# albertfgu/diffwave-sashimi

Hardware: AMD Instinct MI355X
Metric: audio samples/sec (generate.py-style reverse-diffusion sampling, T=200) (higher is better)
Workload: dtype f32-equivalent (3-term bf16 split, 6 products, fp32 accumulate); 1 GPU; wnet_h256_d36_T200; backbone=wavenet, batch_per_gpu=16, L=16000, T=200, parallelism=independent clips per GPU, no collective, sampler=hipGraph replay, on-device Philox noise

## Files before the change

diffwave-sashimi_amd/csrc/wavenet.h:

```cpp
#pragma once
#include "dws_common.h"

namespace dws {

constexpr int WN_LAYER_KC = 32;
constexpr int WN_BX3_KC = 16;

struct WnLayerArgs {
    const float* x_in;
    float* x_out;
    float* skip;
    const float* part_t;
    int part_t_bstride;
    const float* A1;
    const float* A2;
    const float* Abt;
    int abt_bstride;
    const int* step_idx;
    int abt_tstride, part_t_tstride;
    const float* Wd;
    const float* Wr;
    const float* Ws;
    const float* bias1;
    const float* bias2;
// ... 18 lines not shown
    float scale;
    int B, L, Cout;
    int af_scaled;
};

int launch_fold_weight_norm(const float* v, const float* g, float* out, int O, int inner, hipStream_t s);
int launch_permute_dconv(const float* w, float* out, int C, int KC, hipStream_t s);
int launch_pack_a_frag(const float* w, float* out, int M, int K, hipStream_t s);
int launch_pack_a_frag_t(const float* w, float* out, int O, int K, hipStream_t s);
int launch_step_embed(const float* steps, const float* freq, float* emb, int B, int half, hipStream_t s);
int launch_iota_f32(float* out, int n, hipStream_t s);
int launch_linear_rows(const float* in, const float* W, const float* bias, float* out, int B, int K, int O,
                       int act, hipStream_t s, float* pre_out = nullptr);
int launch_init_conv_bwd_data(const float* g, const float* y, const float* W, float* daudio, int B, int Cin, int C, int L,
                              hipStream_t s);
int launch_init_conv(const float* audio, const float* W, const float* bias, float* x, int B, int Cin, int C, int L,
                     hipStream_t s);
int launch_wn_bias_tap(const float* Wd_all, const float* part_t, float* Abt, int NL, int B, int C, hipStream_t s);
bool wn_layer_mfma_supported(int C, int S);
int launch_wn_layer_mfma(int C, int S, const WnLayerArgs& a, hipStream_t s);
int launch_wn_layer_generic(int C, int S, const WnLayerArgs& a, hipStream_t s);
bool wn_final_mfma_supported(int S);
bool wn_layer_wino_supported(int C, int S);
int launch_wino_dconv(const float* w, float* out, int C, hipStream_t s);
int launch_wn_wino_bias(const float* Wd_all, const float* part_t, float* Abt, int NL, int B, int C, hipStream_t s);
int launch_wn_layer_wino(int C, int S, const WnLayerArgs& a, hipStream_t s);
bool wn_layer_bf16x3_supported(int C, int S);
int launch_wn_layer_bf16x3(int C, int S, const WnLayerArgs& a, hipStream_t s);
int launch_pack_a_bf16x3(const float* w, void* out, int M, int K, hipStream_t s);
int launch_wn_bias_tap_bf16(const float* Wd_all, const float* part_t, const float* bias1_all, void* Abt, int NL, int B, int C,
                            hipStream_t s);
enum { WN_SPLIT_BF16X6 = 0, WN_SPLIT_F16X3 = 1 };
inline int wn_split_terms(int split) { return split == WN_SPLIT_F16X3 ? 2 : 3; }
enum { WN_BX6_MFMA_32 = 0, WN_BX6_MFMA_G2_16 = 1, WN_BX6_MFMA_16 = 2 };
constexpr int WN_BX6_MFMA_DEFAULT = WN_BX6_MFMA_16;
bool wn_layer_bx6_supported(int C, int S);
bool wn_layer_bx6_mfma16_supported(int C, int S, int split);
int launch_wn_layer_bx6(int C, int S, const WnLayerArgs& a, int split, int mfma, hipStream_t s);
int launch_weight_scale(const float* w, size_t n, const float* bias, int nb, const float* bias_b, int nb_b, float* out, hipStream_t s);
int launch_pack_a1_bx6(const float* w, void* out, int C, int split, const float* scale, hipStream_t s);
int launch_pack_a_bx6(const float* w, void* out, int M, int K, int split, const float* scale, hipStream_t s);
int launch_gemm_bx6(const float* A, const float* B, float* C, int M, int N, int K, int split, float sa, float sb, hipStream_t s);
int launch_wn_final(int S, const WnFinalArgs& a, hipStream_t s);

}
```

diffwave-sashimi_amd/csrc/wavenet_bx6.hip:

```cpp
#include <cstdlib>
#include <type_traits>

#include "bf16_split.h"
#include "wavenet.h"
#include "wn_trace.h"

namespace dws {

#ifndef BX6_PF3
#define BX6_PF3 1
#endif
#ifndef BX6_PF2
#define BX6_PF2 2
#endif
#define BX6_PF(NT) ((NT) == 2 ? BX6_PF2 : BX6_PF3)
#ifndef BX6_T_SLOTS
#define BX6_T_SLOTS 0, 2, 3, 4, 6, 7, 9
#endif

typedef float bx6_f32x4 __attribute__((ext_vector_type(4)));

#ifdef BX6_ABL_NO_NT
#define BX6_NT 0
#else
// ... 102 lines not shown
    if (split == WN_SPLIT_F16X3) {
        DWS_CHECK(scale != nullptr, DWS_ERR_INVALID, "pack_a: the fp16 split needs the matrix scale");
        hipLaunchKernelGGL(pack_a_bx6_kernel<SplitF16x2>, dim3(ceil_div(n, 256)), dim3(256), 0, s, w, (unsigned short*)out, M, K, scale);
    } else {
        hipLaunchKernelGGL(pack_a_bx6_kernel<SplitBf16x3>, dim3(ceil_div(n, 256)), dim3(256), 0, s, w, (unsigned short*)out, M, K, scale);
    }
    return DWS_OK;
}

template <int C, int S, int NT>
struct Bx6Tile {
    static constexpr int WAVES = C / 32;
    static constexpr int NTH = WAVES * 64;
    static constexpr int NP = 32;
    static constexpr int KC = (C >= 256) ? 32 : 16;
    static constexpr int NCB = C / KC;
    static constexpr int NKB = C / 16;
    static constexpr int MS = S / C;
    static constexpr int RAW_FLOATS = KC * 4 * NP;
    static constexpr int BOP_BYTES = (KC / 8) * 4 * NT * NP * 16;
    static constexpr int STAGE_FLOATS = 2 * RAW_FLOATS + 2 * BOP_BYTES / 4;
    static constexpr int GATE_BYTES = (C / 8) * NT * 64 * 16;
    static constexpr int MAIN_FLOATS = STAGE_FLOATS > GATE_BYTES / 4 ? STAGE_FLOATS : GATE_BYTES / 4;
    static constexpr int TR_FLOATS = 32 * 64;
    static constexpr int LDS_FLOATS = MAIN_FLOATS + WAVES * TR_FLOATS;
    static constexpr int TITEMS = (KC / 4) * NP * 2;
    static constexpr bool HALVES = WAVES == 8 && NT == 3;
    static constexpr int SW = HALVES ? WAVES / 2 : WAVES;
    static constexpr int NPIECE = KC / (2 * SW);
    static_assert(C % 32 == 0 && S % C == 0 && C % KC == 0 && KC % 16 == 0 && KC % (2 * SW) == 0 && (SW & (SW - 1)) == 0 &&
                  (!HALVES || NCB % 2 == 0) && (TITEMS % NTH == 0) && LDS_FLOATS * 4 <= 163840, "channel counts");
};

enum { BX6_MF_32 = 0, BX6_MF_G2_16 = 1, BX6_MF_16 = 2 };
#ifndef BX6_T16_SLOTS
#define BX6_T16_SLOTS 1, 5, 7, 9, 13, 15, 19
#endif
struct Bx6Nothing {};
template <int MS>
struct Bx6G2State {
    float bias[1 + MS][2];
    bx_f32x4 acc[1 + MS][2][2][2];
};
template <int NT>
__device__ __forceinline__ int bx6_voff_a1h(int lane) { return ((lane >> 5) * (4 * NT * 64) + ((lane >> 4) & 1) * 32 + (lane & 15)) * 16; }
template <typename V8, int NT>
__device__ __forceinline__ void bx6_load_a1h(V8 (&dst)[2][NT], __amdgpu_buffer_rsrc_t r, int voff, int soff) {
#pragma unroll
    for (int h = 0; h < 2; ++h)
#pragma unroll
        for (int t = 0; t < NT; ++t) dst[h][t] = __builtin_bit_cast(V8, __builtin_amdgcn_raw_buffer_load_b128(r, voff + h * 256, soff + t * 1024, 0));
}
template <typename V8, int NT>
struct Bx6G1State {
    float av[2][2][4], ab[2][2];
    bx_f32x4 acc[2][4][2][2];
    V8 ar[2][2][NT];
    int pc[2];
};
template <typename P, int C, int S, bool EXTRA, int MF = BX6_MF_32>
__global__ __launch_bounds__(C * 2, (C >= 128 ? 2 : 1)) void wn_layer_bx6_kernel(WnLayerArgs a, int log2d) {
    using T = Bx6Tile<C, S, P::NT>;
    static_assert(MF == BX6_MF_32 || (P::NT == 3 && !P::SCALED && C == 256 && S == 256), "the 16x16x32 shape: bf16 split, C = S = 256");
    using v8 = typename P::v8;
    using v4 = typename P::v4;
    constexpr int NT = P::NT, NPR = P::NP, NA = 2 * P::NT;
    constexpr int KC = T::KC, MS = T::MS, WAVES = T::WAVES, NCB = T::NCB, NTH = T::NTH, NKB = T::NKB;
    __shared__ __attribute__((aligned(16))) float lds[T::LDS_FLOATS];
    float* const Xraw = lds;
    char* const Bop = reinterpret_cast<char*>(lds + 2 * T::RAW_FLOATS);
    char* const gt = reinterpret_cast<char*>(lds);

    const int tid = threadIdx.x;
    const int lane = tid & 63;
    const int wave = __builtin_amdgcn_readfirstlane(tid >> 6);
    const int l31 = lane & 31, lhi = lane >> 5;
    const int L = a.L, dil = 1 << log2d;
    float* const trw = lds + T::MAIN_FLOATS + wave * T::TR_FLOATS;

    const int nblk = (L + 2 * dil - 1) >> (log2d + 1);
    const int ntl = ((nblk << log2d) + 31) >> 5;
    const int tile = xcd_remap(blockIdx.x, gridDim.x);
    const int b = __builtin_amdgcn_readfirstlane(tile / ntl);
    const int tic = tile % ntl;
#ifdef WN_TILE_ORDER_LINEAR
    const int q0 = __builtin_amdgcn_readfirstlane(tic * 32);
#else
    const int q0 = __builtin_amdgcn_readfirstlane(log2d >= 6 ? ((tic % nblk) << log2d) + (tic / nblk) * 32 : tic * 32);
#endif
    const int q = q0 + l31;
    const int p = ((q >> log2d) << (log2d + 1)) + (q & (dil - 1));

    const float* __restrict__ xb = a.x_in + (size_t)b * C * L;
    unsigned long long* __restrict__ trc = a.trace ? a.trace + ((size_t)blockIdx.x * WAVES + wave) * 32 : nullptr;
    auto stamp = [&](int i) {
        if (trc) {
            const unsigned long long t = __builtin_amdgcn_s_memtime();
            if (lane == 0) trc[i] = t;
        }
    };
// ... 132 lines not shown
#pragma unroll
                for (int e = 0; e < 2; ++e) {
                    const float da = ts.d[k][e][0], d1 = ts.d[k][e][1], d2 = ts.d[k][e][2];
                    if (w == 1) t4[2 * h + e] = (p1 ? d2 : da) - (p1 ? d1 : d2);
                    else t4[2 * h + e] = d1 + (p1 ? -da : d2);
                    if (P::SCALED) t4[2 * h + e] *= P::SX;
                }
                v4 q[NT];
                P::split4(t4, q);
#pragma unroll
                for (int t = 0; t < NT; ++t)
#pragma unroll
                    for (int e = 2 * h; e < 2 * h + 2; ++e) {
                        if (w == 1) ts.pa[k][t][e] = q[t][e];
                        else ts.pb[k][t][e] = q[t][e];
                    }
            }
        }
    };
    auto transform = [&](int c1) {
        TState ts;
#pragma unroll
        for (int u = 0; u < T_UNITS; ++u) transform_unit(c1, u, ts);
    };
    auto keep_residual = [&](int c1) {
        const int ch0 = chunk_of(c1) * KC;
        if (al16 && ch0 / 32 == wave) {
            const float* xs = Xraw + (c1 & 1) * T::RAW_FLOATS;
            const int r0 = ch0 % 32;
#pragma unroll
            for (int i = 0; i < KC / 4; ++i) {
                const int rr = (lane >> 4) + 4 * i;
                const bx6_f32x4 v = *reinterpret_cast<const bx6_f32x4*>(xs + rr * 128 + 32 + 4 * (lane & 15));
                *reinterpret_cast<bx6_f32x4*>(trw + (r0 + rr) * 64 + 4 * (lane & 15)) = v;
            }
        }
    };

    bx_f32x16 acc[2][4];
    __amdgpu_buffer_rsrc_t rA1 = __builtin_amdgcn_make_buffer_rsrc((void*)a.A1, 0, 2 * C * 4 * C * 2 * NT, 0x00020000);
    const int lane16 = lane * 16;
    auto load_a1 = [&](v8 (&dst)[2][NT], int kb, int j) {
#pragma unroll
        for (int m = 0; m < 2; ++m)
#pragma unroll
            for (int t = 0; t < NT; ++t)
#ifdef BX6_ABL_A_HOT
                dst[m][t] = __builtin_bit_cast(v8, __builtin_amdgcn_raw_buffer_load_b128(rA1, lane16, ((mt1[m] * NKB * 4) * NT + t) * 1024 + 0 * (kb + j), 0));
#else
                dst[m][t] = __builtin_bit_cast(v8, __builtin_amdgcn_raw_buffer_load_b128(rA1, lane16, (((mt1[m] * NKB + kb) * 4 + j) * NT + t) * 1024, 0));
#endif
    };

    if (stages(0)) stage_dma(0);
    if (NCB > 1 && stages(1)) stage_dma(1);
    constexpr int PF = BX6_PF(NT);
    v8 a_ring[4][2][NT];
    if constexpr (MF >= BX6_MF_16) {
        static_assert(MF < BX6_MF_16 || (PF == 1 && KC == 32), "one half-step of six fragments ahead: NAF and every vmcnt count as in the 32x32x16 form");
        bx6_load_a1h<v8, NT>(gs1.ar[0], rA1, bx6_voff_a1h<NT>(lane), ((mt1[0] * NKB + 2 * chunk_of(0)) * 4 + 0) * NT * 1024);
    } else {
#pragma unroll
    for (int s0 = 0; s0 < PF; ++s0) load_a1(a_ring[s0], chunk_of(0) * (KC / 16) + (s0 >> 2), s0 & 3);
    }
    constexpr int NAF = PF * NA;
    constexpr int P16 = NPIECE + NAF, P4 = 4 * NPIECE + NAF;
    static_assert(P4 < 64, "vmcnt is a 6-bit counter");
// ... 207 lines not shown
    }
    }
    stamp(2);
    int lane_t = lane;
    if constexpr (MF >= BX6_MF_16) asm volatile("" : "+v"(lane_t));

    [[maybe_unused]] std::conditional_t<MF >= BX6_MF_G2_16, Bx6G2State<MS>, Bx6Nothing> gs2;
    if constexpr (MF >= BX6_MF_G2_16) {
#pragma unroll
        for (int m = 0; m < 1 + MS; ++m)
#pragma unroll
            for (int h = 0; h < 2; ++h) gs2.bias[m][h] = a.bias2[mt2[m] * 32 + 16 * h + (lane_t & 15)];
    }
    const int L4 = L * 4;
    const bool first = a.first_layer, last = a.last_layer;
    __amdgpu_buffer_rsrc_t rXo = __builtin_amdgcn_make_buffer_rsrc((void*)(a.x_out + (size_t)b * C * L), 0, C * L * 4, 0x00020000);
    __amdgpu_buffer_rsrc_t rSk = __builtin_amdgcn_make_buffer_rsrc((void*)(a.skip + (size_t)b * S * L), 0, S * L * 4, 0x00020000);
    const int p0 = ((q0 >> log2d) << (log2d + 1)) + (q0 & (dil - 1));
    int voff4;
    {
        const int n4 = (lane_t & 15) >> 3;
        const int pos4 = (contig ? pbase + 32 * n4 : p0 + n4 * dil) + 4 * (lane_t & 7);
        voff4 = (pos4 < L) ? ((lane_t >> 4) * L + pos4) * 4 : 0x7ffffff0;
    }
    constexpr bool PRELOAD = MS == 1;
    const int voff4s = first ? 0x7ffffff0 : voff4;
    auto load_pre = [&](int m, bx6_f32x4 (&dst)[8]) {
#pragma unroll
        for (int i = 0; i < 8; ++i) {
            if (m == 0) dst[i] = *reinterpret_cast<const bx6_f32x4*>(trw + ((lane_t >> 4) + 4 * i) * 64 + 4 * (lane_t & 15));
            else dst[i] = bx6_load_f4(rSk, voff4s, ((wave * MS + (m - 1)) * 32 + 4 * i) * L4);
        }
    };
    bx6_f32x4 pre[PRELOAD ? 1 + MS : 1][8];
    if (PRELOAD && al16) {
#pragma unroll
        for (int m = 1; m < 1 + MS; ++m) load_pre(m, pre[PRELOAD ? m : 0]);
    }

    const float* melb = (EXTRA && a.melc) ? a.melc + (size_t)(a.mel_bstride ? b : 0) * 2 * C * L : nullptr;
    if constexpr (MF >= BX6_MF_16) {
        const int r16 = lane_t & 15, oct = lane_t >> 4;
#pragma unroll
        for (int c = 0; c < 2; ++c) {
            const int qc = q0 + 16 * c + r16;
            const int pc = ((qc >> log2d) << (log2d + 1)) + (qc & (dil - 1));
            const int gc0 = contig ? pc - pbase : 16 * c + r16, gc1 = contig ? pc - pbase + dil : 32 + 16 * c + r16;
#pragma unroll
            for (int h = 0; h < 2; ++h) {
                float ga[4], gb[4];
#pragma unroll
                for (int e = 0; e < 4; ++e) {
                    const int ch = wave * 32 + 16 * h + 4 * oct + e;
#pragma unroll
                    for (int n = 0; n < 2; ++n) {
                        const int pos = pc + n * dil;
                        float ht, hs;
                        if (n == 0) {
                            ht = (gs1.acc[0][0][h][c][e] + gs1.acc[0][1][h][c][e]) + gs1.acc[0][2][h][c][e];
                            hs = (gs1.acc[1][0][h][c][e] + gs1.acc[1][1][h][c][e]) + gs1.acc[1][2][h][c][e];
                        } else {
                            ht = (gs1.acc[0][1][h][c][e] - gs1.acc[0][2][h][c][e]) - gs1.acc[0][3][h][c][e];
                            hs = (gs1.acc[1][1][h][c][e] - gs1.acc[1][2][h][c][e]) - gs1.acc[1][3][h][c][e];
                        }
                        if (EXTRA && melb && pos < L) {
                            ht += melb[(size_t)ch * L + pos];
                            hs += melb[(size_t)(C + ch) * L + pos];
                        }
// ... 107 lines not shown
            v8 bq[2][NT];
#pragma unroll
            for (int n = 0; n < 2; ++n)
#pragma unroll
                for (int t = 0; t < NT; ++t) bq[n][t] = *reinterpret_cast<const v8*>(gk + (t * 64 + n * 32) * 16);
#pragma unroll
            for (int t = 0; t < NPR; ++t)
#pragma unroll
                for (int m = M0; m < 1 + MS; ++m)
#pragma unroll
                    for (int n = 0; n < 2; ++n)
                        acc2[m][n] = P::mfma(c_cur[m][P::ia(t)], bq[n][P::ib(t)], acc2[m][n]);
#pragma unroll
            for (int m = M0; m < 1 + MS; ++m)
#pragma unroll
                for (int t = 0; t < NT; ++t) c_cur[m][t] = c_nxt[m][t];
        }
    };
    if constexpr (MF >= BX6_MF_G2_16) {
        auto gemm2_16 = [&](auto WITH_RES) {
            const int r16 = lane_t & 15, oct = lane_t >> 4;
            auto& acc2h = gs2.acc;
            constexpr int M0 = decltype(WITH_RES)::value ? 0 : 1;
            const int voffa = (oct >> 1) * (NT * 1024) + ((oct & 1) * 32 + r16) * 16;
            auto load_a2h = [&](v8 (&dst)[1 + MS][NT], int kk, int h) {
#pragma unroll
                for (int m = M0; m < 1 + MS; ++m)
#pragma unroll
                    for (int t = 0; t < NT; ++t)
                        dst[m][t] = __builtin_bit_cast(v8, __builtin_amdgcn_raw_buffer_load_b128(rA2, voffa + h * 256, ((mt2[m] * NKB + 2 * kk) * NT + t) * 1024, 0));
            };
            auto block_of = [&](int kk) { const int k = kk + rot; return k >= NCB ? k - NCB : k; };
            static_assert(KC == 32, "GEMM2's rotation counts 32-channel blocks");
            v8 ah[2][1 + MS][NT];
            load_a2h(ah[0], block_of(0), 0);
            {
                const v8 bf = P::bvals_16(P::SG, 0.f, lane_t);
                const bx_f32x4 zero = {0.f, 0.f, 0.f, 0.f};
#pragma unroll
                for (int m = M0; m < 1 + MS; ++m)
#pragma unroll
                    for (int h = 0; h < 2; ++h) {
                        v8 af[NT];
                        P::rank2_16(gs2.bias[m][h] * ws2, 0.f, lane_t, af);
#pragma unroll
                        for (int n = 0; n < 2; ++n)
#pragma unroll
                            for (int c = 0; c < 2; ++c) {
                                acc2h[m][n][h][c] = zero;
#pragma unroll
                                for (int t = NT - 1; t >= 0; --t) acc2h[m][n][h][c] = P::mfma16(af[t], bf, acc2h[m][n][h][c]);
                            }
                    }
            }
            __syncthreads();
            stamp(4);
            const char* gb = gt + oct * (NT * 64 * 16) + r16 * 16;
#pragma unroll 1
            for (int kk = 0; kk < NCB; ++kk) {
                const char* gk = gb + block_of(kk) * (4 * NT * 64 * 16);
                v8 bq[2][2][NT];
#pragma unroll
                for (int h = 0; h < 2; ++h) {
                    if (h == 0) load_a2h(ah[1], block_of(kk), 1);
                    else load_a2h(ah[0], block_of(kk + 1 < NCB ? kk + 1 : kk), 0);
                    __builtin_amdgcn_sched_barrier(0);
                    if (h == 0) {
#pragma unroll
                        for (int n = 0; n < 2; ++n)
#pragma unroll
                            for (int c = 0; c < 2; ++c)
#pragma unroll
                                for (int t = 0; t < NT; ++t) bq[n][c][t] = *reinterpret_cast<const v8*>(gk + (t * 64 + n * 32 + c * 16) * 16);
                    }
#pragma unroll
                    for (int t = 0; t < NPR; ++t)
#pragma unroll
                        for (int m = M0; m < 1 + MS; ++m)
#pragma unroll
                            for (int n = 0; n < 2; ++n)
#pragma unroll
                                for (int c = 0; c < 2; ++c)
                                    acc2h[m][n][h][c] = P::mfma16(ah[h][m][P::ia(t)], bq[n][c][P::ib(t)], acc2h[m][n][h][c]);
                }
            }
        };
        if (last) gemm2_16(std::false_type{});
        else gemm2_16(std::true_type{});
    } else {
        if (last) gemm2(std::false_type{});
        else gemm2(std::true_type{});
    }
    stamp(5);

    const float rs = 0.70710678118654752440f;
    if (al16) {
#pragma unroll
        for (int m = 0; m < 1 + MS; ++m) {
            if (m == 0 && last) continue;
            if (!PRELOAD || m == 0) load_pre(m, pre[0]);
            asm volatile("s_waitcnt lgkmcnt(0)" ::: "memory");
            if constexpr (MF >= BX6_MF_G2_16) {
                const int r16 = lane_t & 15, oct = lane_t >> 4;
                auto& acc2h = gs2.acc;
#pragma unroll
                for (int n = 0; n < 2; ++n)
#pragma unroll
                    for (int h = 0; h < 2; ++h)
#pragma unroll
                        for (int c = 0; c < 2; ++c)
#pragma unroll
                            for (int r = 0; r < 4; ++r) trw[(16 * h + 4 * oct + r) * 64 + ((n * 32 + 16 * c + r16) ^ (oct << 4))] = acc2h[m][n][h][c][r];
            } else {
#pragma unroll
            for (int n = 0; n < 2; ++n)
#pragma unroll
                for (int r = 0; r < 16; ++r) trw[((r & 3) + 8 * (r >> 2) + 4 * lhi) * 64 + n * 32 + l31] = P::SCALED ? acc2[m][n][r] * inv2 : acc2[m][n][r];
            }
            asm volatile("s_waitcnt lgkmcnt(0)" ::: "memory");
            const int row0 = (m == 0) ? wave * 32 : (wave * MS + (m - 1)) * 32;
#pragma unroll
            for (int i = 0; i < 8; ++i) {
                const bx6_f32x4 v = *reinterpret_cast<const bx6_f32x4*>(trw + ((lane_t >> 4) + 4 * i) * 64 +
                                                                        (MF >= BX6_MF_G2_16 ? (4 * (lane_t & 15)) ^ ((i & 3) << 4) : 4 * (lane_t & 15)));
                bx6_f32x4 o = pre[PRELOAD ? m : 0][i] + v;
                if (m == 0) o = o * rs;
                bx6_store_f4(o, m == 0 ? rXo : rSk, voff4, (row0 + 4 * i) * L4);
                asm volatile("s_nop 1" ::: "memory");
            }
// ... 91 lines not shown
    else hipLaunchKernelGGL((wn_layer_bx6_kernel<P, C, S, false, MF>), dim3(ntiles), dim3(T::NTH), 0, s, a, log2d);
    return DWS_OK;
}

bool wn_layer_bx6_mfma16_supported(int C, int S, int split) { return split == WN_SPLIT_BF16X6 && C == 256 && S == 256; }

bool wn_layer_bx6_supported(int C, int S) {
    return (C == 64 && S == 64) || (C == 128 && S == 128) || (C == 128 && S == 256) || (C == 256 && S == 256);
}

template <typename P>
static int launch_bx6_p(int C, int S, const WnLayerArgs& a, int log2d, hipStream_t s) {
    if (C == 64 && S == 64) return launch_bx6_t<P, 64, 64>(a, log2d, s);
    if (C == 128 && S == 128) return launch_bx6_t<P, 128, 128>(a, log2d, s);
    if (C == 128 && S == 256) return launch_bx6_t<P, 128, 256>(a, log2d, s);
    if (C == 256 && S == 256) return launch_bx6_t<P, 256, 256>(a, log2d, s);
    return set_error(DWS_ERR_UNSUPPORTED, "wn_layer_bx6: (C=%d,S=%d) not instantiated", C, S);
}

int launch_wn_layer_bx6(int C, int S, const WnLayerArgs& a, int split, int mfma, hipStream_t s) {
    int log2d = 0;
    while ((1 << log2d) < a.dilation) ++log2d;
    DWS_CHECK((1 << log2d) == a.dilation, DWS_ERR_UNSUPPORTED, "wn_layer_bx6: dilation %d is not a power of two", a.dilation);
    DWS_CHECK((int64_t)a.L + 4 * (int64_t)a.dilation < ((int64_t)1 << 28), DWS_ERR_UNSUPPORTED, "wn_layer_bx6: L too large");
    DWS_CHECK((int64_t)(C > S ? C : S) * a.L * 4 < ((int64_t)1 << 31), DWS_ERR_UNSUPPORTED,
              "wn_layer_bx6: %d channels x L=%d exceed a 2 GiB tensor per clip", C > S ? C : S, a.L);
    if (split == WN_SPLIT_F16X3) {
        DWS_CHECK(a.hsave == nullptr, DWS_ERR_UNSUPPORTED, "wn_layer_f16x3: the training forward runs with precision=f32 or bf16x6");
        DWS_CHECK(a.wscale != nullptr, DWS_ERR_INVALID, "wn_layer_f16x3: no weight scales");
        return launch_bx6_p<SplitF16x2>(C, S, a, log2d, s);
    }
    if (mfma == WN_BX6_MFMA_G2_16 && wn_layer_bx6_mfma16_supported(C, S, split)) return launch_bx6_t<SplitBf16x3, 256, 256, BX6_MF_G2_16>(a, log2d, s);
    if (mfma == WN_BX6_MFMA_16 && wn_layer_bx6_mfma16_supported(C, S, split)) return launch_bx6_t<SplitBf16x3, 256, 256, BX6_MF_16>(a, log2d, s);
    DWS_CHECK(mfma == WN_BX6_MFMA_32 || mfma == WN_BX6_MFMA_G2_16 || mfma == WN_BX6_MFMA_16, DWS_ERR_INVALID, "wn_layer_bx6: unknown MFMA shape %d", mfma);
    return launch_bx6_p<SplitBf16x3>(C, S, a, log2d, s);
}

template <typename P>
__global__ __launch_bounds__(64) void gemm_bx6_kernel(const float* __restrict__ A, const float* __restrict__ B, float* __restrict__ Cm,
                                                      int M, int N, int K, float sa, float sb) {
    using v8 = typename P::v8;
    const int lane = threadIdx.x, l31 = lane & 31, lhi = lane >> 5;
    const int mt = blockIdx.y, nt = blockIdx.x;
    bx_f32x16 acc;
#pragma unroll
    for (int r = 0; r < 16; ++r) acc[r] = 0.f;
    for (int kb = 0; kb < K / 16; ++kb) {
        v8 af[P::NT], bf[P::NT];
#pragma unroll
        for (int e = 0; e < 8; ++e) {
            const int k = kb * 16 + 8 * lhi + e;
            P::split1(A[(size_t)(mt * 32 + l31) * K + k] * sa, af, e);
            P::split1(B[(size_t)k * N + nt * 32 + l31] * sb, bf, e);
        }
#pragma unroll
        for (int t = 0; t < P::NP; ++t) acc = P::mfma(af[P::ia(t)], bf[P::ib(t)], acc);
    }
    const float inv = 1.f / (sa * sb);
#pragma unroll
    for (int r = 0; r < 16; ++r)
        Cm[(size_t)(mt * 32 + (r & 3) + 8 * (r >> 2) + 4 * lhi) * N + nt * 32 + l31] = acc[r] * inv;
}

int launch_gemm_bx6(const float* A, const float* B, float* Cm, int M, int N, int K, int split, float sa, float sb, hipStream_t s) {
    DWS_CHECK(M > 0 && N > 0 && K > 0 && M % 32 == 0 && N % 32 == 0 && K % 16 == 0, DWS_ERR_UNSUPPORTED,
              "gemm_bf16x6 / gemm_f16x3: M=%d N=%d must be multiples of 32, K=%d of 16", M, N, K);
    if (split == WN_SPLIT_F16X3) {
// ... 25 lines not shown
```

diffwave-sashimi_amd/csrc/wavenet_kernels.hip:

```cpp
#include "dws_common.h"
#include "model.h"
#include "wavenet.h"

namespace dws {

typedef float f32x16 __attribute__((ext_vector_type(16)));


__device__ __forceinline__ void fold_weight_norm_row(const float* __restrict__ v, const float* __restrict__ g,
                                                     float* __restrict__ out, int inner, int o, float* red) {
    const float* vr = v + (size_t)o * inner;
    float s = 0.f;
    for (int i = threadIdx.x; i < inner; i += 256) s += vr[i] * vr[i];
    red[threadIdx.x] = s;
    __syncthreads();
    for (int st = 128; st > 0; st >>= 1) {
        if (threadIdx.x < st) red[threadIdx.x] += red[threadIdx.x + st];
        __syncthreads();
    }
    const float scale = g[o] / sqrtf(red[0]);
    for (int i = threadIdx.x; i < inner; i += 256) out[(size_t)o * inner + i] = vr[i] * scale;
}

__global__ __launch_bounds__(256) void fold_weight_norm_kernel(const float* __restrict__ v, const float* __restrict__ g,
// ... 185 lines not shown
#pragma unroll
        for (int off = 32; off > 0; off >>= 1) acc += __shfl_xor(acc, off);
        if (lane == 0) {
            float y = acc + bo;
            if (pre_out) pre_out[(size_t)b * O + o] = y;
            if (ACT == 1) y = y / (1.f + expf(-y));
            out[(size_t)b * O + o] = y;
        }
    }
}

int launch_linear_rows(const float* in, const float* W, const float* bias, float* out, int B, int K, int O,
                       int act, hipStream_t s, float* pre_out) {
    DWS_CHECK(K <= 1024, DWS_ERR_UNSUPPORTED, "linear_rows: K=%d > 1024 not supported", K);
    dim3 grid(ceil_div(O, 4)), block(256);
    if (act == 1)
        hipLaunchKernelGGL(linear_rows_kernel<1>, grid, block, 0, s, in, W, bias, out, B, K, O, pre_out);
    else
        hipLaunchKernelGGL(linear_rows_kernel<0>, grid, block, 0, s, in, W, bias, out, B, K, O, pre_out);
    return DWS_OK;
}

__global__ void init_conv_kernel(const float* __restrict__ audio, const float* __restrict__ W,
                                 const float* __restrict__ bias, float* __restrict__ x, int Cin, int C, int L) {
    const int b = blockIdx.z, c = blockIdx.y;
    const float bc = bias[c];
    for (int l = blockIdx.x * blockDim.x + threadIdx.x; l < L; l += gridDim.x * blockDim.x) {
        float acc = bc;
        for (int ci = 0; ci < Cin; ++ci) acc = fmaf(W[c * Cin + ci], audio[((size_t)b * Cin + ci) * L + l], acc);
        x[((size_t)b * C + c) * L + l] = dws_relu(acc);
    }
}

int launch_init_conv(const float* audio, const float* W, const float* bias, float* x, int B, int Cin, int C, int L,
                     hipStream_t s) {
    ProfileScope ps("init_conv", s);
    dim3 grid(min(ceil_div(L, 256), 64), C, B);
    hipLaunchKernelGGL(init_conv_kernel, grid, dim3(256), 0, s, audio, W, bias, x, Cin, C, L);
    return DWS_OK;
}

__global__ __launch_bounds__(64) void wn_mask_tail_kernel(float* __restrict__ x, const int32_t* __restrict__ lengths,
                                                          const float* __restrict__ pt, int pt_bstride,
                                                          const int* __restrict__ step_idx, int pt_tstride, int C, int L,
                                                          int reach, size_t row_stride, int div) {
    const int b = blockIdx.y, c = blockIdx.x, lane = threadIdx.x;
    const int len = min(max(lengths[b] / div, 0), L);
    const int end = reach < 0 ? L : (int)min((int64_t)L, (int64_t)len + reach);
    if (len >= end) return;
    const float v = pt ? -pt[(size_t)b * pt_bstride + c + step_row_off(step_idx, pt_tstride)] : 0.f;
    float* row = x + ((size_t)b * C + c) * row_stride;
    const int head = (int)((4 - (((uintptr_t)(row + len) >> 2) & 3)) & 3);
    const int a0 = min(len + head, end);
    const int nvec = (end - a0) >> 2;
    for (int i = len + lane; i < a0; i += 64) row[i] = v;
    float4* q = reinterpret_cast<float4*>(row + a0);
    const float4 v4 = make_float4(v, v, v, v);
    for (int k = lane; k < nvec; k += 64) q[k] = v4;
    for (int i = a0 + 4 * nvec + lane; i < end; i += 64) row[i] = v;
}

int launch_wn_mask_tail(float* x, const int32_t* lengths, int B, int C, int L, int reach, const float* pt, int pt_bstride,
                        const int* step_idx, int pt_tstride, hipStream_t s) {
    ProfileScope ps("wn_mask_tail", s);
    DWS_CHECK(B >= 1 && B <= 65535, DWS_ERR_UNSUPPORTED, "per-clip lengths: B = %d (the grid has one row per clip: 1 .. 65535)", B);
    hipLaunchKernelGGL(wn_mask_tail_kernel, dim3(C, B), dim3(64), 0, s, x, lengths, pt, pt_bstride, step_idx, pt_tstride, C, L, reach,
                       (size_t)L, 1);
    return DWS_OK;
}
// ... 607 lines not shown
```

diffwave-sashimi_amd/csrc/wavenet_model.hip:

```cpp
#include <cmath>

#include "conditioner.h"
#include "model.h"
#include "wavenet.h"
#include "wavenet_backward.h"

namespace dws {

struct WaveNetModel : dws_model {
    int Cin, Cout, C, S, NL, cycle, Ein, Emid, Eout, MB;
    bool cond, mfma_layer, mfma_final;
    bool bf16x3 = false;
    bool bf16x6 = false;
    bool f16x3 = false;
    DevBuf wscale;
    bool wino_opt = true;
    int bx6_mfma = WN_BX6_MFMA_DEFAULT;
    bool bx6_mfma_env_bad = false;
    static bool parse_bx6_mfma(const std::string& v, int& out) {
        if (v == "32x32x16") { out = WN_BX6_MFMA_32; return true; }
        if (v == "gemm2-16x16x32") { out = WN_BX6_MFMA_G2_16; return true; }
        if (v == "16x16x32") { out = WN_BX6_MFMA_16; return true; }
        return false;
    }
    bool wino_fits(int64_t nL) const {
        return (int64_t)std::max(C, S) * nL * 4 < ((int64_t)1 << 31) && nL + 4 * ((int64_t)1 << (cycle - 1)) < ((int64_t)1 << 28);
    }
    bool wino() const { return wino_opt && mfma_layer && !bf16x3 && !bf16x6 && !f16x3 && wn_layer_wino_supported(C, S) && (L == 0 || wino_fits(L)); }
    bool wino_rows() const { return wino() || bf16x6 || f16x3; }

    DevBuf Wi;
    std::vector<DevBuf> A1, Wrs, A2, bias2;
    DevBuf Wd_all;
    DevBuf Abt;
    DevBuf Wt_all, bt_all;
    DevBuf b1_all;
    DevBuf Wf, Af;
    DevBuf freq;
    CopyBatch stack_params, unstack_fc_t;
    bool freq_ready = false;
    DevBuf tmp_pack;
    std::vector<DevBuf> melW0, melW1, melWc;
    DevBuf melc;
    DevBuf mel_u0, mel_u1;
    int64_t melBm = 0;
    DevBuf mel_in;
    int mel_T = 0;
    CondTrainWs cws;
    DevBuf gW0f, gW1f, gWcf;
    DevBuf x0, x1, skip, gate, emb, h1, h2, part_t, scratch_out;
    std::vector<DevBuf> tx, tH;
    std::vector<DevBuf> ATd, ATg;
    std::vector<DevBuf> ATw;
    DevBuf ATf, wpart, bpart;
    bool mfma_bwd = false;
// ... 51 lines not shown
        label_param = "residual_layer.label_embedding.weight";
        A1.resize(NL); Wrs.resize(NL); A2.resize(NL); bias2.resize(NL);
        if (cond) { melW0.resize(NL); melW1.resize(NL); melWc.resize(NL); }
    }

    int set_option(const std::string& key, const std::string& value) override {
        if (key == "precision") {
            if (value == "f32") { bf16x3 = bf16x6 = f16x3 = false; dirty = true; trained_fwd = false; return DWS_OK; }
            if (value == "bf16x3") {
                DWS_CHECK(wn_layer_bf16x3_supported(C, S), DWS_ERR_UNSUPPORTED,
                          "precision=bf16x3 is not built for (res_channels=%d, skip_channels=%d)", C, S);
                bf16x3 = true; bf16x6 = f16x3 = false; dirty = true; trained_fwd = false;
                return DWS_OK;
            }
            if (value == "bf16x6") {
                DWS_CHECK(mfma_layer && wn_layer_bx6_supported(C, S), DWS_ERR_UNSUPPORTED,
                          "precision=bf16x6 is not built for (res_channels=%d, skip_channels=%d)", C, S);
                bf16x6 = true; bf16x3 = f16x3 = false; dirty = true; trained_fwd = false;
                return DWS_OK;
            }
            if (value == "f16x3") {
                DWS_CHECK(mfma_layer && wn_layer_bx6_supported(C, S), DWS_ERR_UNSUPPORTED,
                          "precision=f16x3 is not built for (res_channels=%d, skip_channels=%d)", C, S);
                f16x3 = true; bf16x3 = bf16x6 = false; dirty = true; trained_fwd = false;
                return DWS_OK;
            }
        }
        if (key == "conv_algo") {
            if (value == "winograd") { wino_opt = true; dirty = true; trained_fwd = false; return DWS_OK; }
            if (value == "direct") { wino_opt = false; dirty = true; trained_fwd = false; return DWS_OK; }
        }
        if (key == "bx6_mfma") {
            int v = 0;
            DWS_CHECK(parse_bx6_mfma(value, v), DWS_ERR_INVALID, "bx6_mfma: 32x32x16 | gemm2-16x16x32 | 16x16x32, not '%s'", value.c_str());
            bx6_mfma = v; bx6_mfma_env_bad = false; dirty = true; trained_fwd = false;
            return DWS_OK;
        }
        return dws_model::set_option(key, value);
    }

    float* Wd(int n) const { return Wd_all.f() + (size_t)n * 2 * C * C * 3; }

    int fold(const std::string& p, float* out, int O, int inner, hipStream_t s) {
        return launch_fold_weight_norm(P(p + ".weight_v"), P(p + ".weight_g"), out, O, inner, s);
    }

    int commit(hipStream_t s) override {
        DWS_CHECK(!bx6_mfma_env_bad, DWS_ERR_INVALID, "DWS_BX6_MFMA: 32x32x16 | gemm2-16x16x32 | 16x16x32, not '%s'", std::getenv("DWS_BX6_MFMA") ? std::getenv("DWS_BX6_MFMA") : "");
        DWS_TRY(Wi.ensure((size_t)C * Cin * 4));
        DWS_TRY(fold("init_conv.0.conv", Wi.f(), C, Cin, s));
        DWS_TRY(Wt_all.ensure((size_t)NL * C * Eout * 4));
        DWS_TRY(bt_all.ensure((size_t)NL * C * 4));
        DWS_TRY(b1_all.ensure((size_t)NL * 2 * C * 4));
        DWS_TRY(Wd_all.ensure((size_t)NL * 2 * C * C * 3 * 4));
        if (mfma_layer) DWS_TRY(tmp_pack.ensure((size_t)2 * C * 4 * C * 4));
        stack_params.begin();
        for (int n = 0; n < NL; ++n) {
            const std::string p = "residual_layer.residual_blocks." + std::to_string(n);
            stack_params.add(P(p + ".fc_t.weight"), Wt_all.f() + (size_t)n * C * Eout, (size_t)C * Eout);
            stack_params.add(P(p + ".fc_t.bias"), bt_all.f() + (size_t)n * C, (size_t)C);
            stack_params.add(P(p + ".dilated_conv_layer.conv.bias"), b1_all.f() + (size_t)n * 2 * C, (size_t)2 * C);
            DWS_TRY(fold(p + ".dilated_conv_layer.conv", Wd(n), 2 * C, C * 3, s));
            DWS_TRY(Wrs[n].ensure((size_t)(C + S) * C * 4));
            DWS_TRY(fold(p + ".res_conv", Wrs[n].f(), C, C, s));
            DWS_TRY(fold(p + ".skip_conv", Wrs[n].f() + (size_t)C * C, S, C, s));
            DWS_TRY(bias2[n].ensure((size_t)(C + S) * 4));
            stack_params.add(P(p + ".res_conv.bias"), bias2[n].f(), (size_t)C);
            stack_params.add(P(p + ".skip_conv.bias"), bias2[n].f() + C, (size_t)S);
            if (mfma_layer && (bf16x6 || f16x3)) {
                const int split = f16x3 ? WN_SPLIT_F16X3 : WN_SPLIT_BF16X6;
                const size_t tb = 2 * (size_t)wn_split_terms(split);
                float* sc = nullptr;
                if (f16x3) {
                    DWS_TRY(wscale.ensure((size_t)NL * 2 * 4));
                    sc = wscale.f() + 2 * n;
                    DWS_TRY(launch_weight_scale(Wd(n), (size_t)2 * C * C * 3, P(p + ".dilated_conv_layer.conv.bias"), 2 * C, nullptr, 0, sc, s));
                    DWS_TRY(launch_weight_scale(Wrs[n].f(), (size_t)(C + S) * C, P(p + ".res_conv.bias"), C, P(p + ".skip_conv.bias"), S,
                                                sc + 1, s));
                }
                DWS_TRY(A1[n].ensure((size_t)2 * C * 4 * C * tb));
                DWS_TRY(A2[n].ensure((size_t)(C + S) * C * tb));
// ... 576 lines not shown
```

Baseline: 34060 audio samples/s.

## Add swapped-operand 16x16x32 MFMA variant and vectorized init conv kernel

```diff
diff --git a/diffwave-sashimi_amd/csrc/wavenet.h b/diffwave-sashimi_amd/csrc/wavenet.h
--- a/diffwave-sashimi_amd/csrc/wavenet.h
+++ b/diffwave-sashimi_amd/csrc/wavenet.h
@@ -74,7 +74,7 @@
                             hipStream_t s);
 enum { WN_SPLIT_BF16X6 = 0, WN_SPLIT_F16X3 = 1 };
 inline int wn_split_terms(int split) { return split == WN_SPLIT_F16X3 ? 2 : 3; }
-enum { WN_BX6_MFMA_32 = 0, WN_BX6_MFMA_G2_16 = 1, WN_BX6_MFMA_16 = 2 };
+enum { WN_BX6_MFMA_32 = 0, WN_BX6_MFMA_G2_16 = 1, WN_BX6_MFMA_16 = 2, WN_BX6_MFMA_16S = 3 };
 constexpr int WN_BX6_MFMA_DEFAULT = WN_BX6_MFMA_16;
 bool wn_layer_bx6_supported(int C, int S);
 bool wn_layer_bx6_mfma16_supported(int C, int S, int split);
diff --git a/diffwave-sashimi_amd/csrc/wavenet_bx6.hip b/diffwave-sashimi_amd/csrc/wavenet_bx6.hip
--- a/diffwave-sashimi_amd/csrc/wavenet_bx6.hip
+++ b/diffwave-sashimi_amd/csrc/wavenet_bx6.hip
@@ -158,7 +158,7 @@
                   (!HALVES || NCB % 2 == 0) && (TITEMS % NTH == 0) && LDS_FLOATS * 4 <= 163840, "channel counts");
 };
 
-enum { BX6_MF_32 = 0, BX6_MF_G2_16 = 1, BX6_MF_16 = 2 };
+enum { BX6_MF_32 = 0, BX6_MF_G2_16 = 1, BX6_MF_16 = 2, BX6_MF_16S = 3 };
 #ifndef BX6_T16_SLOTS
 #define BX6_T16_SLOTS 1, 5, 7, 9, 13, 15, 19
 #endif
@@ -192,6 +192,7 @@
     using v4 = typename P::v4;
     constexpr int NT = P::NT, NPR = P::NP, NA = 2 * P::NT;
     constexpr int KC = T::KC, MS = T::MS, WAVES = T::WAVES, NCB = T::NCB, NTH = T::NTH, NKB = T::NKB;
+    constexpr bool SWP = MF == BX6_MF_16S;
     __shared__ __attribute__((aligned(16))) float lds[T::LDS_FLOATS];
     float* const Xraw = lds;
     char* const Bop = reinterpret_cast<char*>(lds + 2 * T::RAW_FLOATS);
@@ -390,7 +391,8 @@
             for (int i = 0; i < KC / 4; ++i) {
                 const int rr = (lane >> 4) + 4 * i;
                 const bx6_f32x4 v = *reinterpret_cast<const bx6_f32x4*>(xs + rr * 128 + 32 + 4 * (lane & 15));
-                *reinterpret_cast<bx6_f32x4*>(trw + (r0 + rr) * 64 + 4 * (lane & 15)) = v;
+                const int cg = SWP ? ((lane & 15) ^ ((r0 + rr) & 15)) : (lane & 15);
+                *reinterpret_cast<bx6_f32x4*>(trw + (r0 + rr) * 64 + 4 * cg) = v;
             }
         }
     };
@@ -664,8 +666,29 @@
             else dst[i] = bx6_load_f4(rSk, voff4s, ((wave * MS + (m - 1)) * 32 + 4 * i) * L4);
         }
     };
+    [[maybe_unused]] int voffp[2][2];
+    if constexpr (SWP) {
+#pragma unroll
+        for (int n = 0; n < 2; ++n)
+#pragma unroll
+            for (int c = 0; c < 2; ++c) {
+                const int posp = (contig ? pbase + 32 * n : p0 + n * dil) + 16 * c + 4 * (lane_t >> 4);
+                voffp[n][c] = (posp < L) ? ((lane_t & 15) * L + posp) * 4 : 0x7ffffff0;
+            }
+    }
     bx6_f32x4 pre[PRELOAD ? 1 + MS : 1][8];
-    if (PRELOAD && al16) {
+    if constexpr (SWP) {
+        static_assert(!SWP || (PRELOAD && MS == 1), "the swapped form preloads its one skip row tile");
+        if (al16) {
+#pragma unroll
+            for (int n = 0; n < 2; ++n)
+#pragma unroll
+                for (int h = 0; h < 2; ++h)
+#pragma unroll
+                    for (int c = 0; c < 2; ++c)
+                        pre[PRELOAD ? 1 : 0][(n * 2 + h) * 2 + c] = bx6_load_f4(rSk, first ? 0x7ffffff0 : voffp[n][c], (wave * 32 + 16 * h) * L4);
+        }
+    } else if (PRELOAD && al16) {
 #pragma unroll
         for (int m = 1; m < 1 + MS; ++m) load_pre(m, pre[PRELOAD ? m : 0]);
     }
@@ -839,6 +862,10 @@
             };
             auto block_of = [&](int kk) { const int k = kk + rot; return k >= NCB ? k - NCB : k; };
             static_assert(KC == 32, "GEMM2's rotation counts 32-channel blocks");
+            auto mm = [&](const v8& wf, const v8& gf, const bx_f32x4& c) __attribute__((always_inline)) {
+                if constexpr (SWP) return P::mfma16(gf, wf, c);
+                else return P::mfma16(wf, gf, c);
+            };
             v8 ah[2][1 + MS][NT];
             load_a2h(ah[0], block_of(0), 0);
             {
@@ -856,7 +883,7 @@
                             for (int c = 0; c < 2; ++c) {
                                 acc2h[m][n][h][c] = zero;
 #pragma unroll
-                                for (int t = NT - 1; t >= 0; --t) acc2h[m][n][h][c] = P::mfma16(af[t], bf, acc2h[m][n][h][c]);
+                                for (int t = NT - 1; t >= 0; --t) acc2h[m][n][h][c] = mm(af[t], bf, acc2h[m][n][h][c]);
                             }
                     }
             }
@@ -888,7 +915,7 @@
                             for (int n = 0; n < 2; ++n)
 #pragma unroll
                                 for (int c = 0; c < 2; ++c)
-                                    acc2h[m][n][h][c] = P::mfma16(ah[h][m][P::ia(t)], bq[n][c][P::ib(t)], acc2h[m][n][h][c]);
+                                    acc2h[m][n][h][c] = mm(ah[h][m][P::ia(t)], bq[n][c][P::ib(t)], acc2h[m][n][h][c]);
                 }
             }
         };
@@ -901,7 +928,76 @@
     stamp(5);
 
     const float rs = 0.70710678118654752440f;
-    if (al16) {
+    if constexpr (SWP) {
+        const int r16 = lane_t & 15, oct = lane_t >> 4;
+        auto& acc2h = gs2.acc;
+        if (al16) {
+            bx6_f32x4 xr[8];
+            if (!last) {
+#pragma unroll
+                for (int n = 0; n < 2; ++n)
+#pragma unroll
+                    for (int h = 0; h < 2; ++h)
+#pragma unroll
+                        for (int c = 0; c < 2; ++c)
+                            xr[(n * 2 + h) * 2 + c] = *reinterpret_cast<const bx6_f32x4*>(trw + (16 * h + r16) * 64 + 4 * ((8 * n + 4 * c + oct) ^ r16));
+            }
+#pragma unroll
+            for (int n = 0; n < 2; ++n)
+#pragma unroll
+                for (int h = 0; h < 2; ++h)
+#pragma unroll
+                    for (int c = 0; c < 2; ++c) {
+                        asm volatile("s_nop 1" : "+v"(acc2h[1][n][h][c]) :: "memory");
+                        const bx6_f32x4 o = pre[PRELOAD ? 1 : 0][(n * 2 + h) * 2 + c] + acc2h[1][n][h][c];
+                        bx6_store_f4(o, rSk, voffp[n][c], (wave * 32 + 16 * h) * L4);
+                    }
+            if (!last) {
+#pragma unroll
+                for (int n = 0; n < 2; ++n)
+#pragma unroll
+                    for (int h = 0; h < 2; ++h)
+#pragma unroll
+                        for (int c = 0; c < 2; ++c) {
+                            asm volatile("s_nop 1" : "+v"(acc2h[0][n][h][c]) :: "memory");
+                            const bx6_f32x4 o = (xr[(n * 2 + h) * 2 + c] + acc2h[0][n][h][c]) * rs;
+                            bx6_store_f4(o, rXo, voffp[n][c], (wave * 32 + 16 * h) * L4);
+                        }
+            }
+            asm volatile("s_nop 1" ::: "memory");
+        } else {
+#pragma unroll
+            for (int n = 0; n < 2; ++n)
+#pragma unroll
+                for (int c = 0; c < 2; ++c) {
+                    int voffe[4];
+#pragma unroll
+                    for (int e = 0; e < 4; ++e) {
+                        const int qc = q0 + 16 * c + 4 * oct + e;
+                        const int pos = ((qc >> log2d) << (log2d + 1)) + (qc & (dil - 1)) + n * dil;
+                        voffe[e] = (pos < L) ? (r16 * L + pos) * 4 : 0x7ffffff0;
+                    }
+#pragma unroll
+                    for (int h = 0; h < 2; ++h) {
+                        const int s0 = (wave * 32 + 16 * h) * L4;
+                        if (!last) {
+#pragma unroll
+                            for (int e = 0; e < 4; ++e) {
+                                const float x = __builtin_bit_cast(float, __builtin_amdgcn_raw_buffer_load_b32(rXall, voffe[e], s0, 0));
+                                const float v = (x + acc2h[0][n][h][c][e]) * rs;
+                                __builtin_amdgcn_raw_buffer_store_b32(__builtin_bit_cast(unsigned, v), rXo, voffe[e], s0, 0);
+                            }
+                        }
+#pragma unroll
+                        for (int e = 0; e < 4; ++e) {
+                            const float old = first ? 0.f : __builtin_bit_cast(float, __builtin_amdgcn_raw_buffer_load_b32(rSk, voffe[e], s0, 0));
+                            const float v = old + acc2h[1][n][h][c][e];
+                            __builtin_amdgcn_raw_buffer_store_b32(__builtin_bit_cast(unsigned, v), rSk, voffe[e], s0, 0);
+                        }
+                    }
+                }
+        }
+    } else if (al16) {
 #pragma unroll
         for (int m = 0; m < 1 + MS; ++m) {
             if (m == 0 && last) continue;
@@ -1059,7 +1155,8 @@
     }
     if (mfma == WN_BX6_MFMA_G2_16 && wn_layer_bx6_mfma16_supported(C, S, split)) return launch_bx6_t<SplitBf16x3, 256, 256, BX6_MF_G2_16>(a, log2d, s);
     if (mfma == WN_BX6_MFMA_16 && wn_layer_bx6_mfma16_supported(C, S, split)) return launch_bx6_t<SplitBf16x3, 256, 256, BX6_MF_16>(a, log2d, s);
-    DWS_CHECK(mfma == WN_BX6_MFMA_32 || mfma == WN_BX6_MFMA_G2_16 || mfma == WN_BX6_MFMA_16, DWS_ERR_INVALID, "wn_layer_bx6: unknown MFMA shape %d", mfma);
+    if (mfma == WN_BX6_MFMA_16S && wn_layer_bx6_mfma16_supported(C, S, split)) return launch_bx6_t<SplitBf16x3, 256, 256, BX6_MF_16S>(a, log2d, s);
+    DWS_CHECK(mfma == WN_BX6_MFMA_32 || mfma == WN_BX6_MFMA_G2_16 || mfma == WN_BX6_MFMA_16 || mfma == WN_BX6_MFMA_16S, DWS_ERR_INVALID, "wn_layer_bx6: unknown MFMA shape %d", mfma);
     return launch_bx6_p<SplitBf16x3>(C, S, a, log2d, s);
 }
 
diff --git a/diffwave-sashimi_amd/csrc/wavenet_kernels.hip b/diffwave-sashimi_amd/csrc/wavenet_kernels.hip
--- a/diffwave-sashimi_amd/csrc/wavenet_kernels.hip
+++ b/diffwave-sashimi_amd/csrc/wavenet_kernels.hip
@@ -241,9 +241,33 @@
     }
 }
 
+constexpr int IC4_ROWS = 8;
+__global__ __launch_bounds__(256) void init_conv4_kernel(const float* __restrict__ audio, const float* __restrict__ W,
+                                                         const float* __restrict__ bias, float* __restrict__ x, int Cin, int C, int L) {
+    const int b = blockIdx.z, c0 = blockIdx.y * IC4_ROWS;
+    const int l = (blockIdx.x * blockDim.x + threadIdx.x) * 4;
+    if (l >= L) return;
+    const float* ab = audio + (size_t)b * Cin * L + l;
+    for (int c = c0; c < min(c0 + IC4_ROWS, C); ++c) {
+        const float bc = bias[c];
+        float4 acc = make_float4(bc, bc, bc, bc);
+        for (int ci = 0; ci < Cin; ++ci) {
+            const float w = W[c * Cin + ci];
+            const float4 a = *reinterpret_cast<const float4*>(ab + (size_t)ci * L);
+            acc.x = fmaf(w, a.x, acc.x); acc.y = fmaf(w, a.y, acc.y); acc.z = fmaf(w, a.z, acc.z); acc.w = fmaf(w, a.w, acc.w);
+        }
+        *reinterpret_cast<float4*>(x + ((size_t)b * C + c) * L + l) = make_float4(dws_relu(acc.x), dws_relu(acc.y), dws_relu(acc.z), dws_relu(acc.w));
+    }
+}
+
 int launch_init_conv(const float* audio, const float* W, const float* bias, float* x, int B, int Cin, int C, int L,
                      hipStream_t s) {
     ProfileScope ps("init_conv", s);
+    if (L % 4 == 0 && (((size_t)audio | (size_t)x) & 15) == 0) {
+        dim3 grid(ceil_div(L / 4, 256), ceil_div(C, IC4_ROWS), B);
+        hipLaunchKernelGGL(init_conv4_kernel, grid, dim3(256), 0, s, audio, W, bias, x, Cin, C, L);
+        return DWS_OK;
+    }
     dim3 grid(min(ceil_div(L, 256), 64), C, B);
     hipLaunchKernelGGL(init_conv_kernel, grid, dim3(256), 0, s, audio, W, bias, x, Cin, C, L);
     return DWS_OK;
diff --git a/diffwave-sashimi_amd/csrc/wavenet_model.hip b/diffwave-sashimi_amd/csrc/wavenet_model.hip
--- a/diffwave-sashimi_amd/csrc/wavenet_model.hip
+++ b/diffwave-sashimi_amd/csrc/wavenet_model.hip
@@ -21,6 +21,7 @@
         if (v == "32x32x16") { out = WN_BX6_MFMA_32; return true; }
         if (v == "gemm2-16x16x32") { out = WN_BX6_MFMA_G2_16; return true; }
         if (v == "16x16x32") { out = WN_BX6_MFMA_16; return true; }
+        if (v == "16x16x32-swapped") { out = WN_BX6_MFMA_16S; return true; }
         return false;
     }
     bool wino_fits(int64_t nL) const {
@@ -138,7 +139,7 @@
         }
         if (key == "bx6_mfma") {
             int v = 0;
-            DWS_CHECK(parse_bx6_mfma(value, v), DWS_ERR_INVALID, "bx6_mfma: 32x32x16 | gemm2-16x16x32 | 16x16x32, not '%s'", value.c_str());
+            DWS_CHECK(parse_bx6_mfma(value, v), DWS_ERR_INVALID, "bx6_mfma: 32x32x16 | gemm2-16x16x32 | 16x16x32 | 16x16x32-swapped, not '%s'", value.c_str());
             bx6_mfma = v; bx6_mfma_env_bad = false; dirty = true; trained_fwd = false;
             return DWS_OK;
         }
@@ -152,7 +153,7 @@
     }
 
     int commit(hipStream_t s) override {
-        DWS_CHECK(!bx6_mfma_env_bad, DWS_ERR_INVALID, "DWS_BX6_MFMA: 32x32x16 | gemm2-16x16x32 | 16x16x32, not '%s'", std::getenv("DWS_BX6_MFMA") ? std::getenv("DWS_BX6_MFMA") : "");
+        DWS_CHECK(!bx6_mfma_env_bad, DWS_ERR_INVALID, "DWS_BX6_MFMA: 32x32x16 | gemm2-16x16x32 | 16x16x32 | 16x16x32-swapped, not '%s'", std::getenv("DWS_BX6_MFMA") ? std::getenv("DWS_BX6_MFMA") : "");
         DWS_TRY(Wi.ensure((size_t)C * Cin * 4));
         DWS_TRY(fold("init_conv.0.conv", Wi.f(), C, Cin, s));
         DWS_TRY(Wt_all.ensure((size_t)NL * C * Eout * 4));
```

Measured after the change: 34150 audio samples/s (median of 6 runs). Within noise of the previous version (+0.3%).
